# Vanlightly/vsr-tlaplus

Hardware: AMD Instinct MI355X
Metric: distinct states/sec (whole node) + time-to-first-violation, VSR 3-replica (higher is better)
Workload: dtype u64

## Files before the change

### vsr_tlaplus_amd/csrc/host_checker.hpp

```cpp
#pragma once

struct PassDst {
  u64* words = nullptr;
  u64 words_cap = 0;
  u64* off = nullptr;
  u64* fp = nullptr;
  u64 cap = 0;
  bool own_words = true;
  bool own_index = true;
};
struct DeepLevelRec { u64 n_new = 0, n_local = 0, generated = 0, max_bag = 0, frontier = 0; };
struct vsrmc_checker {
  vsrmc_model model;
  vsrmc_options opt;
  hipStream_t stream = nullptr;
  hipEvent_t ev[4] = {nullptr, nullptr, nullptr, nullptr};
  Slot* table = nullptr;
  u64 tmask = 0;
  u64* words[2] = {nullptr, nullptr};
  u64* off[2] = {nullptr, nullptr};
  u64* lvl_fp = nullptr;
  u64* pending = nullptr;
  LevelCtl* ctl = nullptr;
  u64* d_find = nullptr;
// ... 151 lines not shown
  int tile;
  u32 ccap;
  int stride;
  size_t lds;
  unsigned blocks_per_cu;
  const void* kernel;
};
FusedShape fused_shape(vsrmc_checker* c, u64 max_bag_of_source, bool plain = false) {
  const Model& M = c->model.M;
  FusedShape f;
  f.stride = (int)std::min<u64>((u64)c->lds_stride, (u64)((M.fixed + (int)std::min<u64>(max_bag_of_source, 255)) | 1));
  const void* kernel = (plain && c->plain_kernel) ? c->plain_kernel : c->fused_kernel;
  const int blk = VSR_BLOCK;
  auto occupancy = [&](int tile, u32 ccap, size_t* lds) {
    *lds = (size_t)tile * f.stride * 8 + 2 * (size_t)ccap * 4;
    int nb = 0;
    if (hipOccupancyMaxActiveBlocksPerMultiprocessor(&nb, kernel, blk, *lds) != hipSuccess) nb = 0;
    return nb;
  };
  f.blk = blk;
  size_t lds64 = 0, lds128 = 0;
  u32 ccap64 = M.R <= 3 ? (u32)VSR_CCAP64 : (u32)VSR_CAND_CAP;
  if (const char* e = std::getenv("VSRMC_CCAP"))
    ccap64 = (u32)std::max(256, std::min(2048, std::atoi(e))) & ~127u;
  const int occ64 = occupancy(64, ccap64, &lds64);
  const bool generic = kernel == (const void*)(ExpandKernel)k_expand<true, 0> || kernel == (const void*)(ExpandKernel)k_expand<true, 1000> ||
                       kernel == (const void*)(ExpandKernel)k_expand<true, 2000>;
  const int occ128 = (M.R <= 3 && generic) ? occupancy(128, 1536u, &lds128) : 0;
  if (M.R <= 3 && occ64 < 3 && occ128 >= 1) {
    f.tile = 128; f.ccap = 1536u; f.lds = lds128; f.blocks_per_cu = (unsigned)std::min(occ128, 2);
  } else {
    f.tile = 64; f.ccap = ccap64; f.lds = lds64; f.blocks_per_cu = (unsigned)std::max(1, std::min(occ64, VSR_OCC + 1));
  }
#if VSR_TILE128
  if (plain && M.R <= 3) {
    size_t l128 = 0;
    const int o128 = occupancy(128, 1024u, &l128);
    if (o128 >= 3) { f.tile = 128; f.ccap = 1024u; f.lds = l128; f.blocks_per_cu = 3; f.kernel = kernel; return f; }
  }
#endif
  f.kernel = kernel;
  if (plain && c->plain5_kernel && M.R <= 3 && f.tile == 64) {
    static const u32 cc5 = std::getenv("VSRMC_CCAP5") ? (u32)std::max(256, std::atoi(std::getenv("VSRMC_CCAP5"))) & ~127u : 896u;
    static const size_t lds5 = std::getenv("VSRMC_LDS5") ? (size_t)std::atoll(std::getenv("VSRMC_LDS5")) : (size_t)31744;
    hipFuncAttributes at;
    size_t dyn = (size_t)64 * f.stride * 8 + 2 * (size_t)cc5 * 4;
    int nb5 = 0;
    if (hipFuncGetAttributes(&at, c->plain5_kernel) == hipSuccess && dyn + at.sharedSizeBytes <= lds5 &&
        hipOccupancyMaxActiveBlocksPerMultiprocessor(&nb5, c->plain5_kernel, blk, dyn) == hipSuccess && nb5 >= VSR_OCC + 1) {
      f.kernel = c->plain5_kernel; f.ccap = cc5; f.lds = dyn; f.blocks_per_cu = (unsigned)(VSR_OCC + 1);
    }
  }
  if (const char* e = std::getenv("VSRMC_MAX_BPC"))
    f.blocks_per_cu = (unsigned)std::max(1, std::min<int>((int)f.blocks_per_cu, std::atoi(e)));
  return f;
}

hipError_t table_alloc(Slot** out, u64 slots) {
  const char* e = std::getenv("VSRMC_TABLE_MEM");
  if (e && std::strcmp(e, "uncached") == 0) return hipExtMallocWithFlags((void**)out, slots * sizeof(Slot), hipDeviceMallocUncached);
  if (e && std::strcmp(e, "finegrained") == 0) return hipExtMallocWithFlags((void**)out, slots * sizeof(Slot), hipDeviceMallocFinegrained);
  return hipMalloc((void**)out, slots * sizeof(Slot));
}

int wset_ensure(vsrmc_checker* c) {
  if (c->opt.world <= 1) return 0;
  if (c->d_wset) {
    if (c->wset_dirty) {
      HIPCHK(hipMemsetAsync(c->h_wset.fp, 0, (c->h_wset.mask + 1) * 8, c->stream));
      HIPCHK(hipMemsetAsync(c->h_wset.epoch, 0, (c->h_wset.mask + 1) * 4, c->stream));
      c->wset_dirty = false;
      c->wepoch = 0;
    }
// ... 779 lines not shown
```

### vsr_tlaplus_amd/csrc/vsr_actions.hpp

```cpp
#pragma once
#include "vsr_model.hpp"

namespace vsr {

#define VSR_NSLOT 6

#ifndef VSR_PACK_DELTA
#define VSR_PACK_DELTA 1
#endif
struct Delta {
  u64 hdr;
  u64 rep[4];
#if VSR_PACK_DELTA
  u32 r : 3;
  u32 action : 5;
  u32 used : 8;
  int err;
  u64 pjw;
  VSR_HD int pj(int s) const { return (int)((pjw >> (8 * s)) & 0xFF) - 1; }
  VSR_HD void set_pj(int s, int j) { pjw = (pjw & ~((u64)0xFF << (8 * s))) | ((u64)(u32)(j + 1) << (8 * s)); }
  VSR_HD void clear_pj() { pjw = 0; }
#else
  int r;
  int action;
// ... 36 lines not shown
}
template <typename PTR>
VSR_HD void bag_send_at(const Model& M, PTR bag, int nmsg, Delta& D, u64 key, const int SLOT) {
#pragma unroll
  for (int k = 0; k < VSR_NSLOT; k++)
    if (((D.used >> k) & 1) && (D.pnew[k] & KEYMASK) == key) {
      int c = m_count(D.pnew[k]) + 1;
      if (c > 3) { D.err = ERR_REP_COUNT; return; }
      D.pnew[k] = m_set_count(D.pnew[k], c);
      return;
    }
  D.used |= 1 << SLOT;
  D.set_pj(SLOT, -1);
  D.pnew[SLOT] = m_set_count(key, 1);
  for (int j0 = 0; j0 < nmsg; j0 += 4) {
    const u64 w0 = bag[j0], w1 = j0 + 1 < nmsg ? bag[j0 + 1] : 0, w2 = j0 + 2 < nmsg ? bag[j0 + 2] : 0, w3 = j0 + 3 < nmsg ? bag[j0 + 3] : 0;
    const bool h0 = (w0 & KEYMASK) == key, h1 = (w1 & KEYMASK) == key, h2 = (w2 & KEYMASK) == key, h3 = (w3 & KEYMASK) == key;
    if (h0 | h1 | h2 | h3) {
      const u64 w = h0 ? w0 : h1 ? w1 : h2 ? w2 : w3;
      int c = m_count(w) + 1;
      if (c > 3) { D.err = ERR_REP_COUNT; c = 3; }
      D.set_pj(SLOT, j0 + (h0 ? 0 : h1 ? 1 : h2 ? 2 : 3));
      D.pnew[SLOT] = m_set_count(w, c);
      return;
    }
  }
}
template <typename PTR>
VSR_HD void bag_send(const Model& M, PTR bag, int nmsg, Delta& D, u64 key) { bag_send_at(M, bag, nmsg, D, key, 1); }
template <typename PTR>
VSR_HD void bag_broadcast(const Model& M, PTR bag, int nmsg, Delta& D, u64 key, int source) {
#pragma unroll
  for (int d = 1; d <= 5; d++)
    if (d <= M.R && d != source) {
      D.used |= 1 << d;
      D.set_pj(d, -1);
      D.pnew[d] = m_set_count(m_set_dest(key, d), 1);
    }
  const u64 nodest = ~((u64)7 << 6);
  for (int j0 = 0; j0 < nmsg; j0 += 4) {
    u64 wq[4];
    wq[0] = bag[j0];
    wq[1] = j0 + 1 < nmsg ? bag[j0 + 1] : 0;
    wq[2] = j0 + 2 < nmsg ? bag[j0 + 2] : 0;
    wq[3] = j0 + 3 < nmsg ? bag[j0 + 3] : 0;
    bool any = false;
#pragma unroll
    for (int u = 0; u < 4; u++) any |= ((wq[u] ^ key) & KEYMASK & nodest) == 0;
    if (!any) continue;
#pragma unroll
    for (int u = 0; u < 4; u++) {
      const u64 w = wq[u];
      if (((w ^ key) & KEYMASK & nodest) != 0) continue;
      const int d = m_dest(w);
      int c = m_count(w) + 1;
      if (c > 3) { D.err = ERR_REP_COUNT; c = 3; }
#pragma unroll
      for (int q = 1; q <= 5; q++)
        if (q == d && ((D.used >> q) & 1)) {
          D.set_pj(q, j0 + u);
          D.pnew[q] = m_set_count(w, c);
        }
    }
  }
  if (D.used & 1) {
#pragma unroll
    for (int q = 1; q <= 5; q++)
      if (((D.used >> q) & 1) && ((D.pnew[q] ^ D.pnew[0]) & KEYMASK) == 0) {
        int c = m_count(D.pnew[0]) + 1;
        if (c > 3) { D.err = ERR_REP_COUNT; c = 3; }
// ... 490 lines not shown
  }
#pragma unroll
  for (int i = 0; i < 6; i++) {
    if (i >= M.np) break;
    const u64 h = hash_msg(M, w, M.pitab[i]);
    d[i] += add ? h : (u64)0 - h;
  }
}
template <typename PTR>
VSR_HD void hash_child(const Model& M, PTR rec, const Delta& D, u64* Hc) {
  PTR pb = rec + 1 + (D.r - 1) * M.wpr;
  u64 dinv = 0;
  u64 d[6] = {0, 0, 0, 0, 0, 0};
  hash_word_delta<0>(M, pb[0], D.rep[0], D.r, dinv, d);
  hash_word_delta<1>(M, pb[1], D.rep[1], D.r, dinv, d);
  if (M.wpr > 2) hash_word_delta<2>(M, pb[2], D.rep[2], D.r, dinv, d);
  if (M.wpr > 3) hash_word_delta<3>(M, pb[3], D.rep[3], D.r, dinv, d);
#pragma unroll
  for (int k = 0; k < VSR_NSLOT; k++)
    if ((D.used >> k) & 1) {
      hash_msg_term(M, D.pnew[k], true, dinv, d);
      if (D.pj(k) >= 0) hash_msg_term(M, rec[M.fixed + D.pj(k)], false, dinv, d);
    }
#pragma unroll
  for (int i = 0; i < 6; i++) {
    if (i >= M.np) break;
    Hc[i] = rec[M.h0 + i] + dinv + d[i];
  }
}

template <typename PTR>
VSR_HD int check_invariants_child(const Model& M, PTR rec, const Delta& D) {
  if (!(M.inv_mask & 3)) return 0;
  int bad = 0;
  const u32 own_log = (u32)D.rep[1];
  for (int v = 0; v < M.n; v++) {
    if (hdr_acked(D.hdr, v) != 2) continue;
    int holders = 0;
    for (int r = 1; r <= M.R; r++) {
      u32 lg = (r == D.r) ? own_log : (u32)rec[1 + (r - 1) * M.wpr + 1];
      bool has = false;
      for (int i = 1; i <= 3; i++) {
        int e = log_byte(lg, i);
        if (e && entry_val(e) == v) has = true;
      }
      holders += has ? 1 : 0;
    }
    if ((M.inv_mask & 1) && holders == 0) bad |= 1;
    if ((M.inv_mask & 2) && !(holders >= M.R / 2 + 1)) bad |= 2;
  }
  return bad;
}

VSR_HD int ord_count(const Model& M, int nmsg) { return M.m0 + nmsg * (M.R + 1); }

}
```

### vsr_tlaplus_amd/csrc/vsr_kernels.hpp

```cpp
#pragma once
#include <hip/hip_runtime.h>

#include "vsr_actions.hpp"
#include "vrst_actions.hpp"
#include "vras_actions.hpp"

namespace vsr {

template <int MODEL>
struct ModelOps;
template <>
struct ModelOps<0> {
  template <bool GUARD_ONLY, typename PTR>
  static VSR_HD bool gen_(const Model& M, PTR rec, int ord, Delta& D) { return gen<GUARD_ONLY>(M, rec, ord, D); }
  template <typename PTR>
  static VSR_HD u32 guard_pre(const Model& M, PTR rec, u64 hdr, const u64* Areg, int slot, int* kind0, int info) {
    return guard_slot_pre(M, rec, hdr, Areg, slot, kind0, info);
  }
  template <typename PTR>
  static VSR_HD u32 guard(const Model& M, PTR rec, int slot, int* kind0) { return guard_slot(M, rec, slot, kind0); }
  static VSR_HD int other_kind(int) { return A_SendGetState; }
  template <typename PTR>
  static VSR_HD void hash_child_(const Model& M, PTR rec, const Delta& D, u64* Hc) { hash_child(M, rec, D, Hc); }
  template <typename PTR>
// ... 65 lines not shown
  u64 act_generated[16];
  u64 cand_cnt[8];
  u64 rec_words;
  u64 ties;
  u64 phase_cycles[8];
  u64 tile_cursor;
  u64 n_written;
  u64 fp_xor, fp_sum;
  u32 full;
  u32 full_pad_;
  u64 full_info;
  u64 limit_unchecked;
  u64 n_redo, redo_out, redo_cap;
};

__host__ __device__ __forceinline__ int owner_of(u64 fp, int world) { return (int)(((fp >> 40) & 0xFFFFFF) % (u64)world); }

enum { MODE_NORMAL = 0, MODE_PROBE = 1, MODE_INSERT = 2, MODE_REGEN = 3, MODE_NO_FOOTPRINT = 0x100 ,
       MODE_REDO_LIST = 0x200  };
#define VSR_TILE_MAX 128
#define VSR_BLOCK 256
#ifndef VSR_PHASE_CLOCKS
#define VSR_PHASE_CLOCKS 0
#endif
#if VSR_PHASE_CLOCKS
#define VSR_CLK() __builtin_readcyclecounter()
#else
#define VSR_CLK() ((u64)0)
#endif
#define VSR_CAND_CAP 2048
#ifndef VSR_WAVE_DIAG
#define VSR_WAVE_DIAG 0
#endif
#ifndef VSR_TAKE
#define VSR_TAKE 0
#endif
#ifndef VSR_SPEC_CAS
#define VSR_SPEC_CAS 0
#endif
#ifndef VSR_DIRECT_REFS
#define VSR_DIRECT_REFS 1
#endif
#ifndef VSR_NO_TAIL_SYNC
#define VSR_NO_TAIL_SYNC 1
#endif
#ifndef VSR_COPY8
#define VSR_COPY8 0
#endif
#ifndef VSR_TILE128
#define VSR_TILE128 0
#endif
#ifndef VSR_TAKE_BATCH
#define VSR_TAKE_BATCH 512
#endif
#ifndef VSR_TILE_BATCH
#define VSR_TILE_BATCH 4
#endif
#ifndef VSR_REDO
#define VSR_REDO 1
#endif
#ifndef VSR_REFS_AHEAD
#define VSR_REFS_AHEAD 0
#endif
#if (VSR_REFS_AHEAD || VSR_TAKE) && VSR_REDO
#undef VSR_REDO
#define VSR_REDO 0
#endif
#ifndef VSR_COOP_COPY
#define VSR_COOP_COPY 1
#endif

#ifndef VSR_ROUND_REV
#define VSR_ROUND_REV 0
#endif
#if VSR_WAVE_DIAG == 3
#define VSR_SYNC_G(g) do { const u64 b0_ = __builtin_readcyclecounter(); __syncthreads(); if (tid == 64) s_wd[g] += __builtin_readcyclecounter() - b0_; } while (0)
#elif VSR_WAVE_DIAG
#define VSR_SYNC_G(g) do { const u64 b0_ = __builtin_readcyclecounter(); __syncthreads(); if (VSR_WAVE_DIAG == 1 || (g) == 7) wd_wait += __builtin_readcyclecounter() - b0_; } while (0)
#else
#define VSR_SYNC_G(g) __syncthreads()
#endif
#ifndef VSR_OCC
#define VSR_OCC 4
#endif
#ifndef VSR_PROBE_FOOTPRINT
#define VSR_PROBE_FOOTPRINT 1
#endif

__device__ __forceinline__ void raise_error(LevelCtl* ctl, int code, u64 info) {
  if (atomicCAS(&ctl->err, 0u, (u32)code) == 0u) ctl->err_info = info;
}

__device__ __forceinline__ void raise_full(LevelCtl* ctl, u64 info) {
  if (ctl->full == 0u) {
    ctl->full_info = info;
    ctl->full = 1u;
  }
}

struct WSet {
  u64* fp;
  u32* epoch;
  u64 mask;
};
__device__ __forceinline__ u64 wset_home(u64 fp, u64 mask) { return (fp >> 13) & mask; }
__device__ __forceinline__ bool wset_insert(const WSet* w, u64 fp, int level) {
  const u64 mask = w->mask;
// ... 31 lines not shown
__device__ __forceinline__ u64 wave_alloc(u64* counter) {
  u64 active = __ballot(1);
  int lane = lane_id();
  int leader = __ffsll((long long)active) - 1;
  u64 base = 0;
  if (lane == leader) base = atomicAdd((unsigned long long*)counter, (unsigned long long)__popcll(active));
  base = __shfl(base, leader);
  return base + (u64)__popcll(active & (((u64)1 << lane) - 1));
}

struct CntReg {
  u32* p;
  __device__ __forceinline__ void home() const { (*p)++; }
  __device__ __forceinline__ void extra() const { (*p)++; }
};
struct CntLds {
  unsigned long long* p;
  __device__ __forceinline__ void home() const {}
  __device__ __forceinline__ void extra() const { atomicAdd(p, 1ull); }
};
struct Probe {
  u64 slot;
  u64 meta;
  bool claimed;
  bool reload;
  bool full;
};
template <typename CNT>
__device__ __forceinline__ Probe probe_insert(Slot* table, u64 mask, u64 fp, CNT nprobe) {
  typedef u64 u64x2 __attribute__((ext_vector_type(2)));
  Probe r;
  r.slot = 0; r.meta = META_EMPTY; r.claimed = false; r.reload = false; r.full = false;
  u64 i = fp & mask;
#if VSR_SPEC_CAS
  {
    const u64 old = atomicCAS((unsigned long long*)&table[i].fp, 0ull, (unsigned long long)fp);
    const u64x2 sk = *(const u64x2*)&table[i];
    nprobe.home();
    if (old == 0) { r.slot = i; r.claimed = true; return r; }
    if (old == fp) {
      r.slot = i;
      if (sk.x == fp) r.meta = sk.y; else r.reload = true;
      return r;
    }
    i = (i + 1) & mask;
  }
#else
  {
    const u64x2 sk = *(const u64x2*)&table[i];
    nprobe.home();
    u64 cur = sk.x;
    if (cur == 0) {
      cur = atomicCAS((unsigned long long*)&table[i].fp, 0ull, (unsigned long long)fp);
      if (cur == 0) { r.slot = i; r.claimed = true; return r; }
      if (cur == fp) { r.slot = i; r.reload = true; return r; }
    } else if (cur == fp) {
      r.slot = i;
      r.meta = sk.y;
      return r;
    }
    i = (i + 1) & mask;
  }
#endif
  for (u32 lines = 0; lines < 2048; lines++) {
    const u64 lb = i & ~(u64)3;
    const u64x2* lp = (const u64x2*)&table[lb];
    const u64x2 s0 = lp[0], s1 = lp[1], s2 = lp[2], s3 = lp[3];
#pragma unroll
    for (int k = 0; k < 4; k++) {
      if (lb + k < i) continue;
      const u64x2 sk = k == 0 ? s0 : k == 1 ? s1 : k == 2 ? s2 : s3;
      nprobe.extra();
      u64 cur = sk.x;
      if (cur == 0) {
        cur = atomicCAS((unsigned long long*)&table[lb + k].fp, 0ull, (unsigned long long)fp);
        if (cur == 0) {
          r.slot = lb + k;
          r.claimed = true;
          return r;
        }
        if (cur == fp) {
          r.slot = lb + k;
          r.reload = true;
          return r;
        }
        continue;
      }
      if (cur == fp) {
        r.slot = lb + k;
        r.meta = sk.y;
        return r;
      }
    }
    i = (lb + 4) & mask;
  }
  r.full = true;
// ... 91 lines not shown
    }
    M.h0 = 1 + SR * M.wpr;
    M.fixed = M.h0 + M.np + VSR_PAD_WORDS;
    M.pitab[0] = 0x24u;
    if (SN == 2) M.pitab[1] = 0x21u;
    if (SN == 3) { M.pitab[1] = 0x18u; M.pitab[2] = 0x21u; M.pitab[3] = 0x09u; M.pitab[4] = 0x12u; M.pitab[5] = 0x06u; }
  }
}

constexpr int expand_occ(bool fused, int spec, int plain) {
  return !fused ? 3 : spec == 0 ? 2 : (plain == 5 || plain == 6) ? VSR_OCC + 1 : VSR_OCC;
}
template <bool FUSED, int SPEC = 0, int PLAIN = 0, int BLK = VSR_BLOCK>
__global__ void __launch_bounds__(BLK, expand_occ(FUSED, SPEC, PLAIN) / (BLK > VSR_BLOCK ? BLK / VSR_BLOCK : 1))
k_expand(Model Marg, const u64* __restrict__ fr_words, const u64* __restrict__ fr_off, u64 n_parents, int level, int rank,
         Slot* table, u64 tmask, u64* pending, u64 pending_cap, LevelCtl* ctl, int stride, int world_arg, u64* cand_send,
         u64 cand_cap, u32 pchunk ,
         u64* nx_words, u64 nx_words_cap, u64* nx_off, u64 nx_cap, u64* lvl_fp, u32 ichunk, u32 wchunk, int tile, u32 ccap ,
         u64* filter, u64 fmask, u64* cand_idx, u32 cchunk ,
         int mode_arg, u64 p_offset ,
         const WSet* wset, u32 wepoch) {
  constexpr bool IS_PLAIN = PLAIN == 1 || PLAIN == 5;
  const int mode = IS_PLAIN ? (int)MODE_NORMAL : PLAIN == 3 ? (int)MODE_REGEN : PLAIN == 4 ? (int)MODE_INSERT : PLAIN == 6 ? (int)MODE_PROBE : (mode_arg & 0xFF);
  const bool no_footprint = !IS_PLAIN && PLAIN != 6 && (mode_arg & MODE_NO_FOOTPRINT) != 0;
  const int world = PLAIN ? 1 : world_arg;
  Model M = Marg;
  specialise<SPEC>(M, Marg);
  typedef ModelOps<SPEC / 1000> Ops;
  extern __shared__ u64 smem[];
  u64* s_rec = smem;
  u32* s_cand = (u32*)(smem + tile * stride);
  u32* s_cand2 = s_cand + ccap;
  __shared__ u32 s_ncand, s_napply, s_dead, s_maxbag, s_maxbag_out, s_skip, s_nsurv, s_risky, s_ntotal;
  constexpr int TILE_MAX = BLK < VSR_BLOCK ? BLK / 2 : (!VSR_TILE128 && FUSED && SPEC % 1000 != 0 && (SPEC % 1000) / 100 <= 3) ? 64 : VSR_TILE_MAX;
  constexpr bool COOP = VSR_COOP_COPY && FUSED && IS_PLAIN;
  constexpr bool REDO_OK = VSR_REDO && FUSED && (IS_PLAIN || PLAIN == 6);
  __shared__ u32 s_alive[TILE_MAX];
  __shared__ u64 s_ref[TILE_MAX];
  __shared__ u64 s_pfp[TILE_MAX];
  __shared__ u32 s_kcount[16], s_kbase[16];
  __shared__ int s_slotinfo[64];
  __shared__ unsigned long long s_fxs[2];
  __shared__ unsigned long long s_acc[32];
  __shared__ u64 s_chunk_base;
  __shared__ u32 s_chunk_used, s_tile_base, s_tile_cursor;
  __shared__ u64 s_ich_base, s_wch_base;
  __shared__ u32 s_ich_used, s_wch_used, s_tile_ibase, s_tile_wbase, s_tile_icur, s_tile_wcur, s_wneed;
  __shared__ unsigned long long s_cstate[8];
  constexpr bool fused = FUSED;
  constexpr u64 CS_NONE = ((u64)1 << 40) - 1;

  const int tid = threadIdx.x, lane = tid & 63;
#if VSR_WAVE_DIAG
  u64 wd_wait = 0;
  const u64 wd_t0 = __builtin_readcyclecounter();
  __shared__ unsigned long long s_wd[8];
  if (tid < 8) s_wd[tid] = 0;
#endif
  const u64 ntiles = (n_parents + tile - 1) / tile;
  const int tshift = 31 - __clz(tile);
  if (tid < 32) s_acc[tid] = 0;
  if (tid < 2) s_fxs[tid] = 0;
  if (tid == 0) s_maxbag_out = 0;
  if (tid < 64) s_slotinfo[tid] = (SPEC / 1000 == 0 && tid < M.m0) ? slot_info(M, tid) : 0;
  if (tid == 0) {
    s_chunk_base = 0; s_chunk_used = pchunk;
    s_ich_base = 0; s_ich_used = ichunk; s_wch_base = 0; s_wch_used = wchunk;
  }
  if (tid < 8) s_cstate[tid] = (CS_NONE << 24) | cchunk;
  VSR_SYNC_G(0);

  __shared__ u64 s_tile_cur;
  u64 my_next = 0;
#if VSR_TAKE
  __shared__ u32 s_tile_n;
  u32 my_take = (u32)tile, my_n = 0, avg_q8 = 0;
  __shared__ u64 s_take_end;
  if (tid == 0) {
    my_next = atomicAdd((unsigned long long*)&ctl->tile_cursor, (unsigned long long)VSR_TAKE_BATCH);
    s_take_end = my_next + VSR_TAKE_BATCH;
    my_n = my_take;
  }
#elif VSR_REFS_AHEAD
  __shared__ u64 s_tile_nxt;
  __shared__ u64 s_ref2[TILE_MAX];
  u64 my_next2 = 0;
  if (tid == 0) {
    my_next = atomicAdd((unsigned long long*)&ctl->tile_cursor, 1ull);
    my_next2 = atomicAdd((unsigned long long*)&ctl->tile_cursor, 1ull);
    s_tile_nxt = my_next;
  }
  VSR_SYNC_G(0);
  if (tid < tile) {
    const u64 i0 = s_tile_nxt * (u64)tile + (u64)tid;
    s_ref2[tid] = (s_tile_nxt < ntiles && i0 < n_parents) ? fr_off[i0] : 0;
  }
  VSR_SYNC_G(0);
#else
  __shared__ u32 s_tile_left;
  const u32 tbatch = ntiles >= (u64)gridDim.x * 16 ? (u32)VSR_TILE_BATCH : 1u;
  if (tid == 0) { my_next = atomicAdd((unsigned long long*)&ctl->tile_cursor, 1ull) * (u64)tbatch; s_tile_left = tbatch - 1; }
#endif
  __shared__ u32 s_over;
  if (tid == 0) s_over = 0;
  for (;;) {
    if (tid == 0) {
      s_tile_cur = my_next;
#if VSR_REFS_AHEAD
      s_tile_nxt = my_next2;
      my_next = my_next2;
      if (my_next2 < ntiles) my_next2 = atomicAdd((unsigned long long*)&ctl->tile_cursor, 1ull);
    }
    if (0) {
#endif
#if VSR_TAKE
      s_tile_n = my_n;
      if (my_next < n_parents) {
        const u64 end = s_take_end;
        my_next += my_n;
        if (my_next >= end) { my_next = atomicAdd((unsigned long long*)&ctl->tile_cursor, (unsigned long long)VSR_TAKE_BATCH); s_take_end = my_next + VSR_TAKE_BATCH; my_n = my_take; }
        else { const u64 room = end - my_next; my_n = (room < (u64)my_take + 8 && room <= (u64)tile) ? (u32)room : my_take; }
      }
#else
      if (my_next < ntiles) {
        const u32 left = s_tile_left;
        if (left) { my_next++; s_tile_left = left - 1; }
        else { my_next = atomicAdd((unsigned long long*)&ctl->tile_cursor, 1ull) * (u64)tbatch; s_tile_left = tbatch - 1; }
      }
#endif
    }
    const u64 t_0 = VSR_CLK();
    if (tid == 0) { s_ncand = 0; s_dead = 0; s_maxbag = 0; s_wneed = 0; s_skip = 0; s_nsurv = 0; s_over = 0; if (!IS_PLAIN) s_risky = 0; }
    if (tid < tile) s_alive[tid] = 0;
    if (tid < 16) s_kcount[tid] = 0;
    VSR_SYNC_G(0);
    u64 tile_i = s_tile_cur;
    tile_i = ((u64)(u32)__builtin_amdgcn_readfirstlane((int)(u32)(tile_i >> 32)) << 32) | (u32)__builtin_amdgcn_readfirstlane((int)(u32)tile_i);
#if VSR_TAKE
    if (tile_i >= n_parents) break;
    const u64 p_base = tile_i;
    const int np_tile = (int)((n_parents - p_base) < (u64)s_tile_n ? (n_parents - p_base) : (u64)s_tile_n);
#else
    if (tile_i >= ntiles) break;
    u64 p_base = tile_i * (u64)tile;
    int np_tile = (int)((n_parents - p_base) < (u64)tile ? (n_parents - p_base) : (u64)tile);
    if constexpr (REDO_OK) {
      if (mode_arg & MODE_REDO_LIST) {
        const u64 e = ((const u64*)p_offset)[tile_i >> 1];
        const int cnt = (int)(e >> 48);
        int half = 1;
        while (half * 2 < cnt) half *= 2;
        p_base = (e & (((u64)1 << 48) - 1)) + ((tile_i & 1) ? (u64)half : 0);
        np_tile = (tile_i & 1) ? cnt - half : half;
      }
      p_base = ((u64)(u32)__builtin_amdgcn_readfirstlane((int)(u32)(p_base >> 32)) << 32) | (u32)__builtin_amdgcn_readfirstlane((int)(u32)p_base);
      np_tile = __builtin_amdgcn_readfirstlane(np_tile);
    }
#endif
    u32 cbits[2] = {0u, 0u};
    if constexpr (PLAIN == 3) {
      const int pm = tid & (tile - 1), gg = tid >> tshift, GG = BLK >> tshift;
      if (pm < np_tile) {
        const u32* row = (const u32*)filter + (p_offset + p_base + (u64)pm) * fmask;
#pragma unroll
        for (int q = 0; q < 2; q++)
          if ((u64)(gg + q * GG) < fmask) cbits[q] = row[gg + q * GG];
      }
    }

#if VSR_REFS_AHEAD
    u64 ref_pre = 0;
    if (tid < tile) {
      const u64 i1 = s_tile_nxt * (u64)tile + (u64)tid;
      if (s_tile_nxt < ntiles && i1 < n_parents) ref_pre = fr_off[i1];
    }
#endif
    if (tid < np_tile) {
#if VSR_REFS_AHEAD
      const u64 ref = s_ref2[tid];
#else
      const u64 ref = fr_off[p_base + tid];
#endif
      s_ref[tid] = ref;
      if (ref) atomicMax(&s_maxbag, (u32)((int)(ref & 255) - M.fixed));
      if ((int)(ref & 255) > stride) raise_error(ctl, ERR_INTERNAL, (p_base + (u64)tid) << 16);
    }
#if !VSR_DIRECT_REFS
    VSR_SYNC_G(1);
#endif
    constexpr int SG = BLK / 16;
    for (int half = 0; half < tile; half += 4 * SG)
      for (int wbase = 0; wbase < stride; wbase += 64) {
        u64 v[4][4];
#if VSR_DIRECT_REFS
        u64 refq[4];
#pragma unroll
        for (int q = 0; q < 4; q++) {
          const int p = half + (tid >> 4) + SG * q;
          refq[q] = p < np_tile ? fr_off[p_base + (u64)p] : 0;
        }
#endif
#pragma unroll
        for (int q = 0; q < 4; q++) {
          const int p = half + (tid >> 4) + SG * q;
#if VSR_DIRECT_REFS
          const u64 ref = refq[q];
#else
          const u64 ref = p < np_tile ? s_ref[p] : 0;
#endif
          const u64 off = ref >> 8;
          const int len = (int)(ref & 255) < stride ? (int)(ref & 255) : stride;
#pragma unroll
          for (int j = 0; j < 4; j++) {
            const int k = wbase + (tid & 15) + 16 * j;
            v[q][j] = k < len ? fr_words[off + k] : 0;
          }
        }
#pragma unroll
        for (int q = 0; q < 4; q++) {
          const int p = half + (tid >> 4) + SG * q;
#if VSR_DIRECT_REFS
          const int len = (int)(refq[q] & 255) < stride ? (int)(refq[q] & 255) : stride;
#else
          const int len = p < np_tile ? ((int)(s_ref[p] & 255) < stride ? (int)(s_ref[p] & 255) : stride) : 0;
#endif
#pragma unroll
          for (int j = 0; j < 4; j++) {
            const int k = wbase + (tid & 15) + 16 * j;
            if (k < len) s_rec[p * stride + k] = v[q][j];
          }
        }
      }
#if VSR_REFS_AHEAD
    if (tid < tile) s_ref2[tid] = ref_pre;
#endif
    VSR_SYNC_G(2);
    if (tid < np_tile && s_ref[tid] != 0) {
      const u64* r0 = s_rec + tid * stride;
      u64 pf;
      u32 pa;
      canonical_fp(M, r0[0], r0 + M.h0, &pf, &pa);
      s_pfp[tid] = pf;
    }

    const u64 t_1 = VSR_CLK();
    {
      const int nslots = M.m0 + (int)s_maxbag;
      const int nitems = nslots << tshift;
      const int p_mine = tid & (tile - 1);
      const bool mine_valid = p_mine < np_tile && s_ref[p_mine] != 0;
      const u64* rec_mine = s_rec + p_mine * stride;
      u64 Areg[6] = {0, 0, 0, 0, 0, 0};
      u64 hdr_mine = 0;
      if (mine_valid) {
        hdr_mine = rec_mine[0];
#pragma unroll
        for (int r = 1; r <= 5; r++)
          if (r <= M.R) Areg[r] = rec_mine[1 + (r - 1) * M.wpr];
      }
      const u32 PRIV = PLAIN == 6 ? 0u : (ccap - (u32)BLK) / BLK;
      const u32 shared0 = PRIV * BLK;
      for (u32 k = tid; k < ccap; k += BLK) s_cand[k] = ~0u;
      VSR_SYNC_G(3);
      u32 nmine = 0;
      bool alive = false;
      if constexpr (SPEC / 1000 == 0) {
        auto emit = [&](int kind, int p, int ord) {
          atomicAdd(&s_kcount[kind], 1u);
// ... 136 lines not shown
        if constexpr (REDO_OK) {
          if (np_tile > 1) {
            const u64 k = atomicAdd((unsigned long long*)&ctl->n_redo, 1ull);
            if (k < ctl->redo_cap) { ((u64*)ctl->redo_out)[k] = p_base | ((u64)np_tile << 48); listed = true; s_over = 1; }
          }
        }
        if (!listed) raise_error(ctl, ERR_FRONTIER_FULL, p_base);
      }
      u32 acc = 0;
      if constexpr (!IS_PLAIN && FUSED && VSR_PROBE_FOOTPRINT) {
        const u32 keep = (mode == MODE_PROBE && !no_footprint) ? Ops::probe_actions() : ~0u;
        for (int a = 0; a < 16; a++)
          if ((keep >> a) & 1u) {
            s_kbase[a] = acc;
            acc += s_kcount[a];
          }
        s_napply = acc > ccap ? ccap : acc;
        if (keep != ~0u) {
          for (int a = 0; a < 16; a++)
            if (!((keep >> a) & 1u)) {
              s_kbase[a] = acc;
              acc += s_kcount[a];
            }
          if (!s_over && (s_risky || (int)s_maxbag + M.R - 1 > M.max_bag)) s_acc[15] += acc - s_napply;
        }
      } else {
        for (int a = 0; a < 16; a++) {
          s_kbase[a] = acc;
          acc += s_kcount[a];
        }
      }
      s_ncand = acc > ccap ? ccap : acc;
      if constexpr (PLAIN == 6) { s_ntotal = acc; s_ncand = s_napply; }
#if VSR_TAKE
      {
        const u32 q8 = (acc << 8) / (u32)np_tile;
        avg_q8 = avg_q8 ? (3u * avg_q8 + q8) >> 2 : q8;
        const u32 want = avg_q8 ? ((u32)VSR_TAKE << 8) / avg_q8 : (u32)tile;
        my_take = want < 8u ? 8u : want > (u32)tile ? (u32)tile : want;
      }
#endif
      if (fused) s_wneed = s_ncand * (u32)(M.fixed + (int)s_maxbag + 5);
    }
    const u64 t_2 = VSR_CLK();
    VSR_SYNC_G(6);
    const u32 ncand = s_ncand;
    if constexpr (REDO_OK) {
      if (s_over) {
        VSR_SYNC_G(6);
        continue;
      }
    }
    for (u32 c = tid; c < ccap; c += BLK) {
      const u32 code = s_cand[c];
      if (code == ~0u) continue;
      const u32 pos = atomicAdd(&s_kbase[code >> 18], 1u);
      if (pos < ccap) s_cand2[pos] = code;
    }
    VSR_SYNC_G(6);

    const u64 t_3 = VSR_CLK();
    if (fused && (mode == MODE_NORMAL || mode == MODE_REGEN)) {
      if (s_ich_used + ncand > ichunk) {
        const u32 used = s_ich_used;
        const u64 base = s_ich_base;
        for (u32 k = used + tid; k < ichunk; k += BLK) {
          nx_off[base + k] = 0;
          lvl_fp[base + k] = 0;
        }
        VSR_SYNC_G(6);
        if (tid == 0) {
          u64 nb = atomicAdd((unsigned long long*)&ctl->n_new, (unsigned long long)ichunk);
          if (nb + ichunk > nx_cap) { raise_full(ctl, nb); nb = 0; }
          s_ich_base = nb;
// ... 5 lines not shown
        VSR_SYNC_G(6);
        if (tid == 0) {
          u64 nb = atomicAdd((unsigned long long*)&ctl->words_new, (unsigned long long)wchunk);
          if (nb + wchunk > nx_words_cap) { raise_full(ctl, nb); nb = 0; }
          if (s_wneed > wchunk) { raise_error(ctl, ERR_FRONTIER_FULL, p_base); s_skip = 1; }
          s_wch_base = nb;
          s_wch_used = 0;
        }
        VSR_SYNC_G(6);
      }
      if (tid == 0) { s_tile_ibase = s_ich_used; s_tile_wbase = s_wch_used; s_tile_icur = 0; s_tile_wcur = 0; }
    } else
    if (!fused && s_chunk_used + ncand > pchunk) {
      const u32 used = s_chunk_used;
      const u64 base = s_chunk_base;
      for (u32 k = used + tid; k < pchunk && used < pchunk; k += BLK) pending[3 * (base + k) + 1] = ~(u64)0;
      VSR_SYNC_G(6);
      if (tid == 0) {
        u64 nb = atomicAdd((unsigned long long*)&ctl->n_pending, (unsigned long long)pchunk);
        if (nb + pchunk > pending_cap) {
          raise_error(ctl, ERR_FRONTIER_FULL, nb);
          nb = 0;
        }
        s_chunk_base = nb;
        s_chunk_used = 0;
      }
      VSR_SYNC_G(6);
    }
    const u32 ncand_apply = s_skip ? 0u : ((!IS_PLAIN && FUSED && VSR_PROBE_FOOTPRINT) ? s_napply : ncand);
    constexpr bool dd_on = false;
    if (tid == 0) { s_tile_base = s_chunk_used; s_tile_cursor = 0; }
    VSR_SYNC_G(6);
    const CntLds my_probes{&s_acc[2]};
#if VSR_ROUND_REV
    for (u32 c0 = 0; c0 < ncand_apply; c0 += BLK) {
      const u32 c = c0 + (((c0 / BLK) & 1u) ? (u32)(BLK - 1 - tid) : (u32)tid);
      if (c >= ncand_apply) continue;
#else
    for (u32 c = tid; c < ncand_apply; c += BLK) {
#endif
      const u32 code = s_cand2[c];
      const int p = (int)((code >> 11) & 127), ord = (int)(code & 2047);
      const u64* rec = s_rec + p * stride;
      Delta D;
      const u64 a_0 = VSR_CLK();
      if (!Ops::template gen_<false>(M, rec, ord, D) || D.action != (int)(code >> 18)) {
        raise_error(ctl, ERR_INTERNAL, ((p_base + (u64)p) << 16) | (u64)ord);
        continue;
      }
      if (D.err) {
        raise_error(ctl, D.err, ((p_base + (u64)p) << 16) | (u64)ord);
        continue;
      }
      if constexpr (PLAIN == 6) {
        if (Ops::invariants(M, rec, D) != 0) {
          const u64 i = atomicAdd((unsigned long long*)&ctl->n_pending, 1ull);
          if (i < pending_cap) { pending[2 * i] = origin_make(p_base + (u64)p, ord); pending[2 * i + 1] = 0; }
        }
        continue;
      }
      const u64 a_1 = VSR_CLK();
      if (!IS_PLAIN && fused && mode == MODE_PROBE && Ops::invariants(M, rec, D) == 0) continue;
      u64 Hc[6];
      Ops::hash_child_(M, rec, D, Hc);
      u64 fp;
      u32 ak;
      canonical_fp(M, D.hdr, Hc, &fp, &ak);
      const u64 key = meta_make(level, ak, s_pfp[p]);
      const u64 a_2 = VSR_CLK();
      if (tid == 0) { s_acc[10] += a_1 - a_0; s_acc[11] += a_2 - a_1; }
      if (!fused && world > 1) {
        const int owner = owner_of(fp, world);
        if (owner != rank) {
          for (int o = 0; o < world; o++)
            if (owner == o) {
              u64 i = wave_alloc(&ctl->cand_cnt[o]);
              if (i < cand_cap) {
                cand_send[2 * ((u64)o * cand_cap + i)] = fp;
                cand_send[2 * ((u64)o * cand_cap + i) + 1] = key;
                cand_idx[(u64)o * cand_cap + i] = origin_make(p_offset + p_base + (u64)p, ord);
              } else {
                raise_error(ctl, ERR_FRONTIER_FULL, i);
              }
            }
          continue;
        }
// ... 73 lines not shown
          atomicAdd(&s_acc[9], 1ull);
          atomicXor(&s_fxs[0], (unsigned long long)fp);
          atomicAdd(&s_fxs[1], (unsigned long long)fp);
          do_write = false;
        }
        const u64 a_3 = VSR_CLK();
        if (tid == 0) s_acc[12] += a_3 - a_2;
        u64 idx = 0;
        u64 dst = 0;
        int plen = 0, clen = 0;
        if (do_write) {
          plen = (int)(s_ref[p] & 255);
          clen = M.fixed + hdr_nmsg(D.hdr);
          const u32 io = atomicAdd(&s_tile_icur, 1u);
          const u32 wo = atomicAdd(&s_tile_wcur, (u32)clen);
          idx = s_ich_base + s_tile_ibase + io;
          dst = s_wch_base + s_tile_wbase + wo;
        }
        if constexpr (COOP) {
          const u64 act = __ballot(1);
          u64 wm = __ballot(do_write);
          const int nact = __popcll(act), rnk = __popcll(act & (((u64)1 << lane) - 1));
          while (wm) {
            const int l0 = __ffsll((long long)wm) - 1;
            wm &= wm - 1;
            const int l1 = wm ? __ffsll((long long)wm) - 1 : l0;
            wm &= wm - 1;
            const int n0 = __builtin_amdgcn_readlane(plen, l0), n1 = l1 != l0 ? __builtin_amdgcn_readlane(plen, l1) : 0;
            const u64* r0 = s_rec + __builtin_amdgcn_readlane(p, l0) * stride;
            const u64* r1 = s_rec + __builtin_amdgcn_readlane(p, l1) * stride;
            u64* o0 = nx_words + readlane64(dst, l0);
            u64* o1 = nx_words + readlane64(dst, l1);
            for (int k = rnk; k < n0 || k < n1; k += nact) {
              const u64 v0 = k < n0 ? r0[k] : 0, v1 = k < n1 ? r1[k] : 0;
              if (k < n0) o0[k] = v0;
              if (k < n1) o1[k] = v1;
            }
          }
        }
        if (do_write) {
          u64* out = nx_words + dst;
          if constexpr (!COOP) {
            typedef u64 u64x2_a8 __attribute__((ext_vector_type(2), aligned(8)));
            int k = 0;
#if VSR_COPY8
            for (; k + 7 < plen; k += 8) {
              u64x2_a8 a0, a1, a2, a3;
              a0.x = rec[k]; a0.y = rec[k + 1]; a1.x = rec[k + 2]; a1.y = rec[k + 3];
              a2.x = rec[k + 4]; a2.y = rec[k + 5]; a3.x = rec[k + 6]; a3.y = rec[k + 7];
              *(u64x2_a8*)(out + k) = a0;
              *(u64x2_a8*)(out + k + 2) = a1;
              *(u64x2_a8*)(out + k + 4) = a2;
              *(u64x2_a8*)(out + k + 6) = a3;
            }
#endif
            if (plen - k >= 2) {
              u64x2_a8 cur;
              cur.x = rec[k];
              cur.y = rec[k + 1];
              for (; k + 3 < plen; k += 2) {
                u64x2_a8 nxt;
                nxt.x = rec[k + 2];
                nxt.y = rec[k + 3];
                *(u64x2_a8*)(out + k) = cur;
                cur = nxt;
              }
              *(u64x2_a8*)(out + k) = cur;
              k += 2;
            }
            for (; k + 1 < plen; k += 2) {
              u64x2_a8 v2;
              v2.x = rec[k];
              v2.y = rec[k + 1];
              *(u64x2_a8*)(out + k) = v2;
            }
            if (k < plen) out[k] = rec[k];
          }
          out[0] = D.hdr;
          u64* ob = out + 1 + (D.r - 1) * M.wpr;
          ob[0] = D.rep[0];
          if (M.wpr > 1) ob[1] = D.rep[1];
          if (M.wpr > 2) ob[2] = D.rep[2];
          if (M.wpr > 3) ob[3] = D.rep[3];
#pragma unroll
          for (int k = 0; k < 6; k++)
            if (k < M.np) out[M.h0 + k] = Hc[k];
          int a = 0;
#pragma unroll
          for (int k = 0; k < VSR_NSLOT; k++)
            if ((D.used >> k) & 1) {
              if (D.pj(k) >= 0) out[M.fixed + D.pj(k)] = D.pnew[k];
              else out[plen + (a++)] = D.pnew[k];
            }
          nx_off[idx] = (dst << 8) | (u64)clen;
          lvl_fp[idx] = fp;
          if (bad && !remote) {
            atomicMin((unsigned long long*)&ctl->viol_fp, (unsigned long long)fp);
            atomicOr(&ctl->viol_mask, (u32)bad);
          }
          if ((u32)hdr_nmsg(D.hdr) > s_maxbag_out) atomicMax(&s_maxbag_out, (u32)hdr_nmsg(D.hdr));
        }
        if (PLAIN == 0 && remote) {
          u64 i = 0;
          for (;;) {
            const unsigned long long old = atomicAdd(&s_cstate[owner], 1ull);
            const u32 pos = (u32)(old & 0xFFFFFFull);
            if (pos == cchunk) {
              u64 nb = atomicAdd((unsigned long long*)&ctl->cand_cnt[owner], (unsigned long long)cchunk);
              if (nb + cchunk > cand_cap) { raise_error(ctl, ERR_FRONTIER_FULL, nb); nb = 0; }
              const u64 ob_ = (u64)(old >> 24);
              (void)ob_;
              i = nb;
              atomicExch(&s_cstate[owner], ((unsigned long long)nb << 24) | 1ull);
              break;
            }
            if (pos < cchunk) {
              i = (u64)(old >> 24) + pos;
              break;
            }
          }
          const u64 e = (u64)owner * cand_cap + i;
          cand_send[2 * e] = fp;
          cand_send[2 * e + 1] = key;
          cand_idx[e] = mode == MODE_REGEN ? origin_make(p_base + (u64)p, ord)
                                           : cand_pack(mode == MODE_INSERT ? (u64)hdr_nmsg(D.hdr) : idx, (u32)bad);
        }
// ... 979 lines not shown
```

### vsr_tlaplus_amd/csrc/vsr_model.hpp

```cpp
#pragma once
#include <stdint.h>

#if defined(__HIPCC__)
#include <hip/hip_runtime.h>
#define VSR_HD __host__ __device__ __forceinline__
#else
#define VSR_HD inline
#endif

#ifndef VSR_PAD_WORDS
#define VSR_PAD_WORDS 0
#endif

namespace vsr {

typedef uint64_t u64;
typedef uint32_t u32;
typedef uint16_t u16;

enum { ST_NORMAL = 0, ST_VIEWCHANGE = 1, ST_RECOVERING = 2 };
enum { T_SVC = 1, T_PREPARE = 2, T_PREPAREOK = 3, T_DVC = 4, T_SV = 5, T_GETSTATE = 6, T_NEWSTATE = 7 };

enum {
  A_Init = 0, A_TimerSendSVC, A_ReceiveHigherSVC, A_ReceiveMatchingSVC, A_SendDVC, A_ReceiveHigherDVC,
// ... 167 lines not shown
}
template <typename PTR>
VSR_HD u64 hash_rep_block(const Model& M, PTR b, int r, u32 pt) {
  u64 h = hash_rep_word<0>(M, b[0], r, pt) + hash_rep_word<1>(M, b[1], r, pt);
  if (M.wpr > 2) h += hash_rep_word<2>(M, b[2], r, pt);
  if (M.wpr > 3) h += hash_rep_word<3>(M, b[3], r, pt);
  return h;
}

VSR_HD u32 auxkey_of(const Model& M, u64 hdr, u32 pt) {
  u32 ak = (u32)hdr_aux_svc(hdr);
  for (int v = 0; v < M.n; v++) ak |= (u32)hdr_acked(hdr, v) << (3 + 2 * ((pt >> (2 * v)) & 3));
  return ak;
}

template <typename PTR>
VSR_HD void hash_full(const Model& M, PTR rec, u64* H) {
  int nmsg = hdr_nmsg(rec[0]);
  for (int i = 0; i < M.np; i++) {
    u32 pt = M.pitab[i];
    u64 sum = 0;
    for (int r = 1; r <= M.R; r++) sum += hash_rep_block(M, rec + 1 + (r - 1) * M.wpr, r, pt);
    for (int j = 0; j < nmsg; j++) sum += hash_msg(M, rec[M.fixed + j], pt);
    H[i] = sum;
  }
}

VSR_HD void canonical_fp(const Model& M, u64 hdr, const u64* H, u64* fp, u32* auxkey) {
  u64 bf = H[0];
  u32 ba = auxkey_of(M, hdr, M.pitab[0]);
#pragma unroll
  for (int i = 1; i < 6; i++) {
    if (i >= M.np) break;
    u64 h = H[i];
    if (h > bf) continue;
    u32 ak = auxkey_of(M, hdr, M.pitab[i]);
    if (h < bf || ak < ba) { bf = h; ba = ak; }
  }
  if (bf == 0) bf = 1;
  *fp = bf;
  *auxkey = ba;
}

static const u64 META_EMPTY = ~(u64)0;
static const u64 META_TAKEN = 1;
static const u64 PFP_MASK = ((u64)1 << 45) - 1;
VSR_HD u64 meta_make(int level, u32 auxkey, u64 parent_fp) {
  return ((u64)level << 55) | ((u64)auxkey << 46) | ((parent_fp & PFP_MASK) << 1);
}
VSR_HD int meta_level(u64 m) { return (int)(m >> 55); }
VSR_HD int meta_auxkey(u64 m) { return (int)((m >> 46) & 511); }
VSR_HD u64 meta_pfp(u64 m) { return (m >> 1) & PFP_MASK; }
constexpr u64 cand_pack(u64 idx, u32 bad) { return idx | ((u64)bad << 56); }
constexpr u64 cand_index(u64 e) { return e & (((u64)1 << 56) - 1); }
constexpr u32 cand_bad(u64 e) { return (u32)(e >> 56); }
static_assert(cand_bad(cand_pack(((u64)1 << 56) - 1, 31)) == 31 && cand_index(cand_pack(((u64)1 << 56) - 1, 31)) == ((u64)1 << 56) - 1 &&
              cand_bad(cand_pack(12345, 16)) == 16 && cand_bad(cand_pack(12345, 4)) == 4 && cand_bad(cand_pack(12345, 6)) == 6,
              "every invariant bit of every model survives the candidate entry");
VSR_HD u64 origin_make(u64 pidx, int ord) { return pidx | ((u64)ord << 40); }
VSR_HD u64 origin_pidx(u64 o) { return o & (((u64)1 << 40) - 1); }
VSR_HD int origin_ord(u64 o) { return (int)(o >> 40); }

}
```

Measured before the change: 1.778 billion.

## Remove dead experimental paths and make several hot loops branch-free

Deletes the unused compile-time experiments (TAKE, SPEC_CAS, REFS_AHEAD, COPY8, TILE128, ROUND_REV) and converts several hot per-thread loops into branchless, predicated code. This covers the broadcast slot setup, the canonical fingerprint minimum, the delta slot writes, and the invariant check, which now packs per-value holder counts into nibbles and returns early when nothing is acked. The cooperative copy now loads without bounds guards, which may read past the record end. A dummy SALU injection knob is added, off by default. The aim is to reduce wave divergence and instruction count, at the risk of extra work in predicated lanes and out-of-bounds loads.

```diff
diff --git a/vsr_tlaplus_amd/csrc/host_checker.hpp b/vsr_tlaplus_amd/csrc/host_checker.hpp
--- a/vsr_tlaplus_amd/csrc/host_checker.hpp
+++ b/vsr_tlaplus_amd/csrc/host_checker.hpp
@@ -207,13 +207,6 @@
   } else {
     f.tile = 64; f.ccap = ccap64; f.lds = lds64; f.blocks_per_cu = (unsigned)std::max(1, std::min(occ64, VSR_OCC + 1));
   }
-#if VSR_TILE128
-  if (plain && M.R <= 3) {
-    size_t l128 = 0;
-    const int o128 = occupancy(128, 1024u, &l128);
-    if (o128 >= 3) { f.tile = 128; f.ccap = 1024u; f.lds = l128; f.blocks_per_cu = 3; f.kernel = kernel; return f; }
-  }
-#endif
   f.kernel = kernel;
   if (plain && c->plain5_kernel && M.R <= 3 && f.tile == 64) {
     static const u32 cc5 = std::getenv("VSRMC_CCAP5") ? (u32)std::max(256, std::atoi(std::getenv("VSRMC_CCAP5"))) & ~127u : 896u;
diff --git a/vsr_tlaplus_amd/csrc/vsr_actions.hpp b/vsr_tlaplus_amd/csrc/vsr_actions.hpp
--- a/vsr_tlaplus_amd/csrc/vsr_actions.hpp
+++ b/vsr_tlaplus_amd/csrc/vsr_actions.hpp
@@ -92,10 +92,11 @@
 VSR_HD void bag_broadcast(const Model& M, PTR bag, int nmsg, Delta& D, u64 key, int source) {
 #pragma unroll
   for (int d = 1; d <= 5; d++)
-    if (d <= M.R && d != source) {
-      D.used |= 1 << d;
-      D.set_pj(d, -1);
-      D.pnew[d] = m_set_count(m_set_dest(key, d), 1);
+    if (d <= M.R) {
+      const bool on = d != source;
+      D.used |= on ? 1u << d : 0u;
+      D.set_pj(d, on ? -1 : D.pj(d));
+      D.pnew[d] = on ? m_set_count(m_set_dest(key, d), 1) : D.pnew[d];
     }
   const u64 nodest = ~((u64)7 << 6);
   for (int j0 = 0; j0 < nmsg; j0 += 4) {
@@ -652,22 +653,29 @@
 template <typename PTR>
 VSR_HD int check_invariants_child(const Model& M, PTR rec, const Delta& D) {
   if (!(M.inv_mask & 3)) return 0;
+  if (!((D.hdr >> 12) & 0x15u & ((1u << (2 * M.n)) - 1))) return 0;
+  const u32 own_log = (u32)D.rep[1];
+  u32 cnt = 0;
+#pragma unroll
+  for (int r = 1; r <= 5; r++) {
+    if (r > M.R) break;
+    const u32 lg = (r == D.r) ? own_log : (u32)rec[1 + (r - 1) * M.wpr + 1];
+    u32 vm = 0;
+#pragma unroll
+    for (int i = 1; i <= 3; i++) {
+      const int e = log_byte(lg, i);
+      vm |= e ? 1u << entry_val(e) : 0u;
+    }
+    cnt += (vm & 1u) | ((vm & 2u) << 3) | ((vm & 4u) << 6) | ((vm & 8u) << 9);
+  }
   int bad = 0;
-  const u32 own_log = (u32)D.rep[1];
-  for (int v = 0; v < M.n; v++) {
-    if (hdr_acked(D.hdr, v) != 2) continue;
-    int holders = 0;
-    for (int r = 1; r <= M.R; r++) {
-      u32 lg = (r == D.r) ? own_log : (u32)rec[1 + (r - 1) * M.wpr + 1];
-      bool has = false;
-      for (int i = 1; i <= 3; i++) {
-        int e = log_byte(lg, i);
-        if (e && entry_val(e) == v) has = true;
-      }
-      holders += has ? 1 : 0;
-    }
-    if ((M.inv_mask & 1) && holders == 0) bad |= 1;
-    if ((M.inv_mask & 2) && !(holders >= M.R / 2 + 1)) bad |= 2;
+#pragma unroll
+  for (int v = 0; v < 4; v++) {
+    if (v >= M.n) break;
+    const int holders = (int)((cnt >> (4 * v)) & 15u);
+    const bool acked = hdr_acked(D.hdr, v) == 2;
+    bad |= (acked && (M.inv_mask & 1) && holders == 0) ? 1 : 0;
+    bad |= (acked && (M.inv_mask & 2) && !(holders >= M.R / 2 + 1)) ? 2 : 0;
   }
   return bad;
 }
diff --git a/vsr_tlaplus_amd/csrc/vsr_kernels.hpp b/vsr_tlaplus_amd/csrc/vsr_kernels.hpp
--- a/vsr_tlaplus_amd/csrc/vsr_kernels.hpp
+++ b/vsr_tlaplus_amd/csrc/vsr_kernels.hpp
@@ -121,47 +121,25 @@
 #ifndef VSR_WAVE_DIAG
 #define VSR_WAVE_DIAG 0
 #endif
-#ifndef VSR_TAKE
-#define VSR_TAKE 0
-#endif
-#ifndef VSR_SPEC_CAS
-#define VSR_SPEC_CAS 0
-#endif
 #ifndef VSR_DIRECT_REFS
 #define VSR_DIRECT_REFS 1
 #endif
 #ifndef VSR_NO_TAIL_SYNC
 #define VSR_NO_TAIL_SYNC 1
 #endif
-#ifndef VSR_COPY8
-#define VSR_COPY8 0
-#endif
-#ifndef VSR_TILE128
-#define VSR_TILE128 0
-#endif
-#ifndef VSR_TAKE_BATCH
-#define VSR_TAKE_BATCH 512
-#endif
 #ifndef VSR_TILE_BATCH
 #define VSR_TILE_BATCH 4
 #endif
 #ifndef VSR_REDO
 #define VSR_REDO 1
 #endif
-#ifndef VSR_REFS_AHEAD
-#define VSR_REFS_AHEAD 0
-#endif
-#if (VSR_REFS_AHEAD || VSR_TAKE) && VSR_REDO
-#undef VSR_REDO
-#define VSR_REDO 0
-#endif
 #ifndef VSR_COOP_COPY
 #define VSR_COOP_COPY 1
 #endif
-
-#ifndef VSR_ROUND_REV
-#define VSR_ROUND_REV 0
-#endif
+#ifndef VSR_DUMMY_SALU
+#define VSR_DUMMY_SALU 0
+#endif
+
 #if VSR_WAVE_DIAG == 3
 #define VSR_SYNC_G(g) do { const u64 b0_ = __builtin_readcyclecounter(); __syncthreads(); if (tid == 64) s_wd[g] += __builtin_readcyclecounter() - b0_; } while (0)
 #elif VSR_WAVE_DIAG
@@ -259,20 +237,6 @@
   Probe r;
   r.slot = 0; r.meta = META_EMPTY; r.claimed = false; r.reload = false; r.full = false;
   u64 i = fp & mask;
-#if VSR_SPEC_CAS
-  {
-    const u64 old = atomicCAS((unsigned long long*)&table[i].fp, 0ull, (unsigned long long)fp);
-    const u64x2 sk = *(const u64x2*)&table[i];
-    nprobe.home();
-    if (old == 0) { r.slot = i; r.claimed = true; return r; }
-    if (old == fp) {
-      r.slot = i;
-      if (sk.x == fp) r.meta = sk.y; else r.reload = true;
-      return r;
-    }
-    i = (i + 1) & mask;
-  }
-#else
   {
     const u64x2 sk = *(const u64x2*)&table[i];
     nprobe.home();
@@ -288,7 +252,6 @@
     }
     i = (i + 1) & mask;
   }
-#endif
   for (u32 lines = 0; lines < 2048; lines++) {
     const u64 lb = i & ~(u64)3;
     const u64x2* lp = (const u64x2*)&table[lb];
@@ -446,7 +409,7 @@
   u32* s_cand = (u32*)(smem + tile * stride);
   u32* s_cand2 = s_cand + ccap;
   __shared__ u32 s_ncand, s_napply, s_dead, s_maxbag, s_maxbag_out, s_skip, s_nsurv, s_risky, s_ntotal;
-  constexpr int TILE_MAX = BLK < VSR_BLOCK ? BLK / 2 : (!VSR_TILE128 && FUSED && SPEC % 1000 != 0 && (SPEC % 1000) / 100 <= 3) ? 64 : VSR_TILE_MAX;
+  constexpr int TILE_MAX = BLK < VSR_BLOCK ? BLK / 2 : (FUSED && SPEC % 1000 != 0 && (SPEC % 1000) / 100 <= 3) ? 64 : VSR_TILE_MAX;
   constexpr bool COOP = VSR_COOP_COPY && FUSED && IS_PLAIN;
   constexpr bool REDO_OK = VSR_REDO && FUSED && (IS_PLAIN || PLAIN == 6);
   __shared__ u32 s_alive[TILE_MAX];
@@ -486,62 +449,19 @@
 
   __shared__ u64 s_tile_cur;
   u64 my_next = 0;
-#if VSR_TAKE
-  __shared__ u32 s_tile_n;
-  u32 my_take = (u32)tile, my_n = 0, avg_q8 = 0;
-  __shared__ u64 s_take_end;
-  if (tid == 0) {
-    my_next = atomicAdd((unsigned long long*)&ctl->tile_cursor, (unsigned long long)VSR_TAKE_BATCH);
-    s_take_end = my_next + VSR_TAKE_BATCH;
-    my_n = my_take;
-  }
-#elif VSR_REFS_AHEAD
-  __shared__ u64 s_tile_nxt;
-  __shared__ u64 s_ref2[TILE_MAX];
-  u64 my_next2 = 0;
-  if (tid == 0) {
-    my_next = atomicAdd((unsigned long long*)&ctl->tile_cursor, 1ull);
-    my_next2 = atomicAdd((unsigned long long*)&ctl->tile_cursor, 1ull);
-    s_tile_nxt = my_next;
-  }
-  VSR_SYNC_G(0);
-  if (tid < tile) {
-    const u64 i0 = s_tile_nxt * (u64)tile + (u64)tid;
-    s_ref2[tid] = (s_tile_nxt < ntiles && i0 < n_parents) ? fr_off[i0] : 0;
-  }
-  VSR_SYNC_G(0);
-#else
   __shared__ u32 s_tile_left;
   const u32 tbatch = ntiles >= (u64)gridDim.x * 16 ? (u32)VSR_TILE_BATCH : 1u;
   if (tid == 0) { my_next = atomicAdd((unsigned long long*)&ctl->tile_cursor, 1ull) * (u64)tbatch; s_tile_left = tbatch - 1; }
-#endif
   __shared__ u32 s_over;
   if (tid == 0) s_over = 0;
   for (;;) {
     if (tid == 0) {
       s_tile_cur = my_next;
-#if VSR_REFS_AHEAD
-      s_tile_nxt = my_next2;
-      my_next = my_next2;
-      if (my_next2 < ntiles) my_next2 = atomicAdd((unsigned long long*)&ctl->tile_cursor, 1ull);
-    }
-    if (0) {
-#endif
-#if VSR_TAKE
-      s_tile_n = my_n;
-      if (my_next < n_parents) {
-        const u64 end = s_take_end;
-        my_next += my_n;
-        if (my_next >= end) { my_next = atomicAdd((unsigned long long*)&ctl->tile_cursor, (unsigned long long)VSR_TAKE_BATCH); s_take_end = my_next + VSR_TAKE_BATCH; my_n = my_take; }
-        else { const u64 room = end - my_next; my_n = (room < (u64)my_take + 8 && room <= (u64)tile) ? (u32)room : my_take; }
-      }
-#else
       if (my_next < ntiles) {
         const u32 left = s_tile_left;
         if (left) { my_next++; s_tile_left = left - 1; }
         else { my_next = atomicAdd((unsigned long long*)&ctl->tile_cursor, 1ull) * (u64)tbatch; s_tile_left = tbatch - 1; }
       }
-#endif
     }
     const u64 t_0 = VSR_CLK();
     if (tid == 0) { s_ncand = 0; s_dead = 0; s_maxbag = 0; s_wneed = 0; s_skip = 0; s_nsurv = 0; s_over = 0; if (!IS_PLAIN) s_risky = 0; }
@@ -550,11 +470,6 @@
     VSR_SYNC_G(0);
     u64 tile_i = s_tile_cur;
     tile_i = ((u64)(u32)__builtin_amdgcn_readfirstlane((int)(u32)(tile_i >> 32)) << 32) | (u32)__builtin_amdgcn_readfirstlane((int)(u32)tile_i);
-#if VSR_TAKE
-    if (tile_i >= n_parents) break;
-    const u64 p_base = tile_i;
-    const int np_tile = (int)((n_parents - p_base) < (u64)s_tile_n ? (n_parents - p_base) : (u64)s_tile_n);
-#else
     if (tile_i >= ntiles) break;
     u64 p_base = tile_i * (u64)tile;
     int np_tile = (int)((n_parents - p_base) < (u64)tile ? (n_parents - p_base) : (u64)tile);
@@ -570,7 +485,6 @@
       p_base = ((u64)(u32)__builtin_amdgcn_readfirstlane((int)(u32)(p_base >> 32)) << 32) | (u32)__builtin_amdgcn_readfirstlane((int)(u32)p_base);
       np_tile = __builtin_amdgcn_readfirstlane(np_tile);
     }
-#endif
     u32 cbits[2] = {0u, 0u};
     if constexpr (PLAIN == 3) {
       const int pm = tid & (tile - 1), gg = tid >> tshift, GG = BLK >> tshift;
@@ -582,19 +496,8 @@
       }
     }
 
-#if VSR_REFS_AHEAD
-    u64 ref_pre = 0;
-    if (tid < tile) {
-      const u64 i1 = s_tile_nxt * (u64)tile + (u64)tid;
-      if (s_tile_nxt < ntiles && i1 < n_parents) ref_pre = fr_off[i1];
-    }
-#endif
     if (tid < np_tile) {
-#if VSR_REFS_AHEAD
-      const u64 ref = s_ref2[tid];
-#else
       const u64 ref = fr_off[p_base + tid];
-#endif
       s_ref[tid] = ref;
       if (ref) atomicMax(&s_maxbag, (u32)((int)(ref & 255) - M.fixed));
       if ((int)(ref & 255) > stride) raise_error(ctl, ERR_INTERNAL, (p_base + (u64)tid) << 16);
@@ -645,9 +548,6 @@
           }
         }
       }
-#if VSR_REFS_AHEAD
-    if (tid < tile) s_ref2[tid] = ref_pre;
-#endif
     VSR_SYNC_G(2);
     if (tid < np_tile && s_ref[tid] != 0) {
       const u64* r0 = s_rec + tid * stride;
@@ -850,14 +750,6 @@
       }
       s_ncand = acc > ccap ? ccap : acc;
       if constexpr (PLAIN == 6) { s_ntotal = acc; s_ncand = s_napply; }
-#if VSR_TAKE
-      {
-        const u32 q8 = (acc << 8) / (u32)np_tile;
-        avg_q8 = avg_q8 ? (3u * avg_q8 + q8) >> 2 : q8;
-        const u32 want = avg_q8 ? ((u32)VSR_TAKE << 8) / avg_q8 : (u32)tile;
-        my_take = want < 8u ? 8u : want > (u32)tile ? (u32)tile : want;
-      }
-#endif
       if (fused) s_wneed = s_ncand * (u32)(M.fixed + (int)s_maxbag + 5);
     }
     const u64 t_2 = VSR_CLK();
@@ -929,13 +821,7 @@
     if (tid == 0) { s_tile_base = s_chunk_used; s_tile_cursor = 0; }
     VSR_SYNC_G(6);
     const CntLds my_probes{&s_acc[2]};
-#if VSR_ROUND_REV
-    for (u32 c0 = 0; c0 < ncand_apply; c0 += BLK) {
-      const u32 c = c0 + (((c0 / BLK) & 1u) ? (u32)(BLK - 1 - tid) : (u32)tid);
-      if (c >= ncand_apply) continue;
-#else
     for (u32 c = tid; c < ncand_apply; c += BLK) {
-#endif
       const u32 code = s_cand2[c];
       const int p = (int)((code >> 11) & 127), ord = (int)(code & 2047);
       const u64* rec = s_rec + p * stride;
@@ -949,6 +835,13 @@
         raise_error(ctl, D.err, ((p_base + (u64)p) << 16) | (u64)ord);
         continue;
       }
+#if VSR_DUMMY_SALU
+      {
+        u32 x = (u32)__builtin_amdgcn_readfirstlane(ord);
+#pragma unroll
+        for (int i = 0; i < VSR_DUMMY_SALU; i++) asm volatile("s_add_u32 %0, %0, 1" : "+s"(x) : : "scc");
+      }
+#endif
       if constexpr (PLAIN == 6) {
         if (Ops::invariants(M, rec, D) != 0) {
           const u64 i = atomicAdd((unsigned long long*)&ctl->n_pending, 1ull);
@@ -1088,7 +981,7 @@
             u64* o0 = nx_words + readlane64(dst, l0);
             u64* o1 = nx_words + readlane64(dst, l1);
             for (int k = rnk; k < n0 || k < n1; k += nact) {
-              const u64 v0 = k < n0 ? r0[k] : 0, v1 = k < n1 ? r1[k] : 0;
+              const u64 v0 = r0[k], v1 = r1[k];
               if (k < n0) o0[k] = v0;
               if (k < n1) o1[k] = v1;
             }
@@ -1099,17 +992,6 @@
           if constexpr (!COOP) {
             typedef u64 u64x2_a8 __attribute__((ext_vector_type(2), aligned(8)));
             int k = 0;
-#if VSR_COPY8
-            for (; k + 7 < plen; k += 8) {
-              u64x2_a8 a0, a1, a2, a3;
-              a0.x = rec[k]; a0.y = rec[k + 1]; a1.x = rec[k + 2]; a1.y = rec[k + 3];
-              a2.x = rec[k + 4]; a2.y = rec[k + 5]; a3.x = rec[k + 6]; a3.y = rec[k + 7];
-              *(u64x2_a8*)(out + k) = a0;
-              *(u64x2_a8*)(out + k + 2) = a1;
-              *(u64x2_a8*)(out + k + 4) = a2;
-              *(u64x2_a8*)(out + k + 6) = a3;
-            }
-#endif
             if (plen - k >= 2) {
               u64x2_a8 cur;
               cur.x = rec[k];
@@ -1143,11 +1025,13 @@
             if (k < M.np) out[M.h0 + k] = Hc[k];
           int a = 0;
 #pragma unroll
-          for (int k = 0; k < VSR_NSLOT; k++)
-            if ((D.used >> k) & 1) {
-              if (D.pj(k) >= 0) out[M.fixed + D.pj(k)] = D.pnew[k];
-              else out[plen + (a++)] = D.pnew[k];
-            }
+          for (int k = 0; k < VSR_NSLOT; k++) {
+            const int j = D.pj(k);
+            u64* const pw = j >= 0 ? out + M.fixed + j : out + plen + a;
+            const bool on = (D.used >> k) & 1;
+            a += (on && j < 0) ? 1 : 0;
+            if (on) *pw = D.pnew[k];
+          }
           nx_off[idx] = (dst << 8) | (u64)clen;
           lvl_fp[idx] = fp;
           if (bad && !remote) {
diff --git a/vsr_tlaplus_amd/csrc/vsr_model.hpp b/vsr_tlaplus_amd/csrc/vsr_model.hpp
--- a/vsr_tlaplus_amd/csrc/vsr_model.hpp
+++ b/vsr_tlaplus_amd/csrc/vsr_model.hpp
@@ -223,10 +223,11 @@
 #pragma unroll
   for (int i = 1; i < 6; i++) {
     if (i >= M.np) break;
-    u64 h = H[i];
-    if (h > bf) continue;
-    u32 ak = auxkey_of(M, hdr, M.pitab[i]);
-    if (h < bf || ak < ba) { bf = h; ba = ak; }
+    const u64 h = H[i];
+    const u32 ak = auxkey_of(M, hdr, M.pitab[i]);
+    const bool take = h < bf || (h == bf && ak < ba);
+    bf = take ? h : bf;
+    ba = take ? ak : ba;
   }
   if (bf == 0) bf = 1;
   *fp = bf;
```

After: 1.798 billion, median of 6. 1.1% higher.
